# yuPeiyu98/Diffusion-Amortized-MCMC

Measured on AMD Instinct MI355X. Metric: Langevin z-steps/sec (B=128, z_dim=128, CIFAR-10), higher is better.
Workload: dtype f32; 1 GPU; cifar10 train-iteration Langevin block: 30 posterior steps on B=128 + 60 prior steps on 2B=256 split over the ranks (value counts posterior z-steps only); global_batch=128, per_rank_batch=128, per_rank_prior_chains=256, z_dim=128, ngf=128, posterior_steps=30, prior_steps=60, parallelism=dp1 (chains sharded, no collective)

## Files before the change

diffusion-amortized-mcmc_amd/csrc/gemm.hip:

```cpp
#include <algorithm>
#include <atomic>
#include <cstdlib>
#include <type_traits>

#include "gemm.h"

namespace damc {

constexpr int BN = 128;

template <int BK, int MT>
struct TileCfg {
  static constexpr int BM = 64 * MT;
  static constexpr int LDA = (BK == 16) ? BM + 2 : BM + 1;
  static constexpr int LDB = BN;
  static constexpr int AQ = BK / 4;
  static constexpr int AROWS_V = BM * BK / 1024;
  static constexpr int AROWS_S = BM * BK / 256;
  static constexpr int BROWS_V = BK / 8;
  static constexpr int BROWS_S = BK / 2;
};

template <int OM>
__device__ __forceinline__ long gemm_row_offset(const GemmArgs& p, int m, int py, int px) {
// ... 849 lines not shown
  hipLaunchKernelGGL((gemm_km_kernel<EPI, OM, PIPE, DBG>), dim3(ntm * ntn, 1, zdim), dim3(256), 0, s, a);
}

static int launch_gemm_km(const GemmArgs& a, Epi epi, OMode om, int zdim, hipStream_t s) {
  const int taps = a.Cg > 0 ? a.K / a.Cg : 0;
  if (!conv_kmajor_ok(a.Cg) || taps * a.Cg != a.K || a.kw <= 0 || taps % a.kw != 0 || taps > 32) return DAMC_ERR_ARG;
  if (om == O_PHASE && zdim != 4) return DAMC_ERR_ARG;
  if (om == O_DENSE && (a.k_per_z <= 0 || a.k_per_z % KM_BK != 0 ||
                        (long)zdim * a.k_per_z < a.K || (long)(zdim - 1) * a.k_per_z >= a.K))
    return DAMC_ERR_ARG;
  if (a.ldb < a.K || ((uintptr_t)a.A | (uintptr_t)a.B) % 16 != 0 || (a.ldb % 4) != 0) return DAMC_ERR_ARG;
  if ((double)a.N * a.ldb * 4 >= 2147483647.0) return DAMC_ERR_UNSUPPORTED;
  const long hwq = (long)a.Hq * a.Wq;
  if (a.M % hwq != 0) return DAMC_ERR_ARG;
  const long img = (long)a.Hin * a.Win * a.Cg;
  const long nimg = a.M / hwq;
  static const long lim = [] {
    const char* e = getenv("DAMC_KM_CHUNK_BYTES");
    const long v = e ? atol(e) : 0;
    return (v > 0 && v < 2147483647L) ? v : 2147483647L;
  }();
  const long per = (lim / 4 - 1) / img;
  if (per < 1) return DAMC_ERR_UNSUPPORTED;
  const long cimg = (om == O_PHASE) ? (long)a.Hout * a.Wout * a.ldc : hwq * a.ldc;
  for (long b0 = 0; b0 < nimg; b0 += per) {
    const long nb = std::min(per, nimg - b0);
    GemmArgs c = a;
    c.A = a.A + b0 * img;
    c.C = a.C + b0 * cimg;
    if (a.mask) c.mask = a.mask + b0 * cimg;
    c.M = (int)(nb * hwq);
    const char* esk = getenv("DAMC_KM_SKINNY");
    const char* ekr = getenv("DAMC_KM_SKINNY_ROWS");
    const int km_rows = ekr ? atoi(ekr) : 64;
    if (epi == EPI_STORE && om == O_DENSE && c.M <= km_rows && c.Hin == 1 && c.Win == 1 && c.Hq == 1 && c.Wq == 1 &&
        c.kw == 1 && c.Cg == c.K && !(esk && esk[0] == '0')) {
      const dim3 g((unsigned)zdim, (unsigned)((c.N + 127) / 128), (unsigned)((c.M + 31) / 32));
      hipLaunchKernelGGL(km_skinny_kernel, g, dim3(256), 0, s, c);
      continue;
    }
#define DAMC_KM(E_, O_)                \
  if (epi == E_ && om == O_) {         \
    launch_km_t<E_, O_>(c, zdim, s);   \
    continue;                          \
  }
    DAMC_KM(EPI_BIAS_ACT, O_PHASE)
    DAMC_KM(EPI_MASK, O_DENSE)
    DAMC_KM(EPI_BIAS_ACT, O_DENSE)
    DAMC_KM(EPI_STORE, O_DENSE)
#undef DAMC_KM
    return DAMC_ERR_UNSUPPORTED;
  }
  return (int)hipGetLastError();
}

constexpr int X3_BM = 256, X3_BN = 128, X3_BK = 32, X3_ROWB = 192;
__device__ __forceinline__ int x3_swz(int row) { return (row >> 1) & 3; }
constexpr int X3_F32A = 2097152, X3A_ROWB = 128;
constexpr int X3_NARROW = 4194304;
constexpr int X3_TAPSHARE = 16777216;
__device__ __forceinline__ int f32a_swz(int r) { return ((r >> 1) & 7) ^ ((((r >> 2) ^ (r >> 3)) & 1) << 1); }
__device__ __forceinline__ int ts_swz(int r) { return ((r >> 1) & 1) | (((r >> 2) & 1) << 2); }
static_assert(X3_NEGK % 32 == 0 && (X3_NEGK & (X3_NEGK - 1)) == 0, "sign blocks are whole K tiles, a power of two");
constexpr int X3_CHUNKS = 12;
typedef __bf16 bf16x8 __attribute__((ext_vector_type(8)));
typedef unsigned int u32x4 __attribute__((ext_vector_type(4)));

constexpr int X3_BASE = 261, X3_RASTER = 16, X3_WIDE = 524288, X3_KREG = 1048576;
constexpr int X3_BITS = X3_BASE | X3_RASTER | X3_WIDE | X3_KREG | X3_F32A | X3_NARROW | X3_TAPSHARE;
__device__ __forceinline__ void split3_octet(const float (&v)[8], bf16x8& h, bf16x8& m, bf16x8& l) {
#pragma unroll
  for (int e = 0; e < 8; ++e) {
    const __bf16 b0 = (__bf16)v[e];
    const float r1 = sub_rn(v[e], (float)b0);
    const __bf16 b1 = (__bf16)r1;
    const float r2 = sub_rn(r1, (float)b1);
    h[e] = b0;
    m[e] = b1;
    l[e] = (__bf16)r2;
  }
}

template <int NT>
__device__ __forceinline__ void proj16(const float* tile, int ts, int r0, int C, const float* w, int ldw,
                                       f32x4 (&acc)[NT]) {
  const int lane = threadIdx.x & 63, m = lane & 15, q = lane >> 4;
#pragma unroll
  for (int t = 0; t < NT; ++t) acc[t] = f32x4{0.f, 0.f, 0.f, 0.f};
  for (int g = 0; g < C / 16; ++g) {
    const f32x4 a = *reinterpret_cast<const f32x4*>(tile + (r0 + m) * ts + 16 * g + 4 * q);
#pragma unroll
    for (int t = 0; t < NT; ++t) {
      const f32x4 b = *reinterpret_cast<const f32x4*>(w + (long)(16 * t + m) * ldw + 16 * g + 4 * q);
#pragma unroll
      for (int e = 0; e < 4; ++e) acc[t] = __builtin_amdgcn_mfma_f32_16x16x4f32(a[e], b[e], acc[t], 0, 0, 0);
    }
  }
}

template <int NT>
__global__ __launch_bounds__(512) void proj_rows_kernel(const float* __restrict__ h, long npix, int C,
                                                        const float* __restrict__ w, int ldw, float* __restrict__ P,
                                                        long pstride) {
  constexpr int TS = 256 + 4;
  __shared__ __attribute__((aligned(16))) float tile[128 * TS];
  const int tid = threadIdx.x, wave = tid >> 6, lane = tid & 63;
  const long p0 = (long)blockIdx.x * 128;
  const int c4 = C / 4;
  for (int i = tid; i < 128 * c4; i += 512) {
    const int r = i / c4, c = (i - r * c4) * 4;
    const long pix = p0 + r;
    *reinterpret_cast<f32x4*>(tile + r * TS + c) =
        pix < npix ? *reinterpret_cast<const f32x4*>(h + pix * C + c) : f32x4{0.f, 0.f, 0.f, 0.f};
  }
  __syncthreads();
  const int m = lane & 15, q = lane >> 4;
  for (int c0 = 0; c0 < C; c0 += PROJ_CHUNK) {
    f32x4 acc[NT];
    proj16<NT>(tile + c0, TS, wave * 16, min(PROJ_CHUNK, C - c0), w + c0, ldw, acc);
    float* Pc = P + (c0 / PROJ_CHUNK) * pstride;
#pragma unroll
    for (int t = 0; t < NT; ++t)
#pragma unroll
      for (int r = 0; r < 4; ++r) {
        const long pix = p0 + wave * 16 + 4 * q + r;
        if (pix < npix) Pc[pix * (16 * NT) + 16 * t + m] = acc[t][r];
      }
  }
}

int launch_proj_rows(const float* h, long npix, int C, const float* w, int ldw, int np, float* P, long pstride,
                     hipStream_t s) {
  if (C <= 0 || C > 256 || C % 16 || (np != 32 && np != 64) || npix <= 0) return DAMC_ERR_ARG;
  if (C > PROJ_CHUNK && pstride < npix * np) return DAMC_ERR_ARG;
  const dim3 grid((unsigned)((npix + 127) / 128));
  if (np == 32)
    hipLaunchKernelGGL(proj_rows_kernel<2>, grid, dim3(512), 0, s, h, npix, C, w, ldw, P, pstride);
  else
    hipLaunchKernelGGL(proj_rows_kernel<4>, grid, dim3(512), 0, s, h, npix, C, w, ldw, P, pstride);
  return (int)hipGetLastError();
}

template <int EPI, int OM, int V = X3_BASE>
__global__ __launch_bounds__(512, (V & X3_NARROW) ? 2 : 1) void gemm_x3_kernel(GemmArgs p) {
  static_assert((V & X3_BASE) == X3_BASE && !(V & ~X3_BITS), "V: X3_BASE and the named variant bits only");
  constexpr bool WIDE = (V & X3_WIDE) != 0;
  constexpr bool NARROW = (V & X3_NARROW) != 0;
  static_assert(!NARROW || !(V & (X3_RASTER | X3_WIDE | X3_KREG | X3_F32A)), "NARROW: the default limb path, unsplit");
  constexpr int BM = WIDE ? 128 : NARROW ? 64 : X3_BM, BN = WIDE ? 256 : X3_BN;
  constexpr bool F32A = (V & X3_F32A) != 0;
  static_assert(!F32A || (OM != O_WGRAD && !WIDE), "F32A: 256 x 128 tiles, not the weight gradient");
  constexpr int AROWB = F32A ? X3A_ROWB : X3_ROWB, ESZ = F32A ? 4 : 6;
  constexpr int AJ = (BM * (F32A ? 8 : X3_CHUNKS) + 511) / 512, BJ = BN * X3_CHUNKS / 512;
  constexpr int BUFB = BM * AROWB + BN * X3_ROWB + ((V & X3_TAPSHARE) ? 2 * X3A_ROWB : 0);
  const int FLOG = __builtin_ctz((unsigned)p.negk >> 5), FLUSH = 1 << FLOG;
  __shared__ __attribute__((aligned(16))) unsigned char smem[2 * (BM + BN) * X3_ROWB];
  const int tid = threadIdx.x;
  const int lane = tid & 63;
  const int wave = tid >> 6;
  const int wm = (WIDE || NARROW) ? wave >> 2 : wave >> 1, wn = (WIDE || NARROW) ? wave & 3 : wave & 1;
  unsigned long long clk_t0 = 0, clk_r0 = 0;
  if (p.clk && tid == 0) {
    clk_t0 = __builtin_amdgcn_s_memtime();
    clk_r0 = __builtin_amdgcn_s_memrealtime();
  }
  constexpr bool RASTER = (V & X3_RASTER) != 0 && OM != O_WGRAD;
  const int wgid = xcd_remap(blockIdx.x, gridDim.x);
  const int ntn = (p.N + BN - 1) / BN;
  int tm, tn, z;
  if constexpr (RASTER) {
    const int nph = OM == O_PHASE ? 4 : 1;
    const int ntm = (p.M + BM - 1) / BM;
    int pr;
    supertile(wgid, ntm, ntn * nph, tm, pr);
    tn = pr / nph;
    z = pr - tn * nph;
  } else {
    tm = wgid / ntn;
    tn = wgid - tm * ntn;
    z = blockIdx.z;
  }
  const int m0 = tm * BM, n0 = tn * BN;

  int pad_y = p.pad_y, pad_x = p.pad_x, py = 0, px = 0;
  const unsigned short* Bg = p.B3;
  const bool KSPLIT = OM != O_WGRAD && p.ksplit > 1;
  constexpr bool KREG = (V & X3_KREG) != 0;
  static_assert(!KREG || !WIDE, "KREG: 256 x 128 tiles only");
  constexpr bool TSHARE = (V & X3_TAPSHARE) != 0;
  static_assert(!TSHARE || F32A, "TAPSHARE: the F32A path (on the slice-major walk)");
  const int nslz = KSPLIT ? p.ksplit / p.kbpw : 1;
  const int zph = KSPLIT ? z / nslz : z, zsl = KSPLIT ? z - zph * nslz : 0;
  if (OM == O_PHASE) {
    py = zph >> 1;
    px = zph & 1;
    pad_y = 1 - py;
    pad_x = 1 - px;
    Bg += (long)zph * p.b_zstride * 3;
  }
  int kbeg = 0, kend = p.K;
  if (KSPLIT) {
    kbeg = zsl * p.k_per_z;
    kend = min(p.K, kbeg + p.k_per_z);
  }
  if constexpr (OM == O_WGRAD) {
    const int nsl = gridDim.z / p.wg_phases;
    const int ph = z / nsl, sl = z - ph * nsl;
    if (p.wg_phases == 4) {
      py = ph >> 1;
      px = ph & 1;
      pad_y = 1 - py;
      pad_x = 1 - px;
    } else {
      pad_y = pad_x = 0;
    }
    Bg += (long)ph * p.b_zstride * 3;
    kbeg = sl * p.k_per_z;
    kend = min(p.K, kbeg + p.k_per_z);
  }
  const int Cg = p.Cg, kw = p.kw, Win = p.Win;
  const int kh = p.K / Cg / kw;
  const int nk = (OM == O_WGRAD || KSPLIT) ? max(kend - kbeg, 0) / X3_BK : p.K / X3_BK;
  const int kt0 = kbeg / X3_BK;
  const int hwq = p.Hq * p.Wq;
  const int nimg = (p.M + hwq - 1) / hwq;
  const __amdgpu_buffer_rsrc_t rsA = __builtin_amdgcn_make_buffer_rsrc(
      F32A ? (void*)p.A : (void*)p.A3, (short)0, (OM == O_WGRAD) ? Cg * p.K * 6 : nimg * p.Hin * Win * Cg * ESZ,
      0x00020000);
  const __amdgpu_buffer_rsrc_t rsB =
      __builtin_amdgcn_make_buffer_rsrc((void*)Bg, (short)0, p.N * p.K * 6, 0x00020000);

  int abase[AJ];
  unsigned amask[AJ], boff[BJ];
#pragma unroll
  for (int j = 0; j < AJ; ++j) {
    const int nch = F32A ? 8 : X3_CHUNKS;
    const int id = tid + 512 * j, row = id / nch, ch = id - row * nch;
    const int m = m0 + row;
    unsigned msk = 0;
    int base = 0;
    if constexpr (OM == O_WGRAD) {
      msk = 0xFFFFFFFFu;
      if (m < p.M) {
        const int t = m / Cg, ci = m - t * Cg;
        const int ty = t / kw, tx = t - ty * kw;
        const int dy = ty - pad_y, dx = tx - pad_x;
        base = ci * p.K + (dy * Win + dx) * p.wg_bp;
        msk = (unsigned)(dy + 1) | ((unsigned)(dx + 1) << 2);
      }
    } else if (m < p.M) {
      const int b = m / hwq;
      const int r = m - b * hwq;
      const int qy = r / p.Wq, qx = r - qy * p.Wq;
      const int iy0 = qy * p.stride - pad_y, ix0 = qx * p.stride - pad_x;
      base = ((b * p.Hin + iy0) * Win + ix0) * Cg;
      for (int ky = 0; ky < kh; ++ky)
        for (int kx = 0; kx < kw; ++kx)
          if ((unsigned)(iy0 + ky) < (unsigned)p.Hin && (unsigned)(ix0 + kx) < (unsigned)Win)
            msk |= 1u << (ky * kw + kx);
    }
    const int q = (ch / 3) ^ x3_swz(row), limb = ch - (ch / 3) * 3;
    abase[j] = F32A ? base * 4 + ((id & 7) ^ f32a_swz(row & 15)) * 16 : base * 6 + q * 48 + limb * 16;
    amask[j] = msk;
  }
#pragma unroll
  for (int j = 0; j < BJ; ++j) {
    const int id = tid + 512 * j, row = id / X3_CHUNKS, ch = id - row * X3_CHUNKS;
    const int q = (ch / 3) ^ x3_swz(row), limb = ch - (ch / 3) * 3;
    boff[j] = (unsigned)((n0 + row) * p.K * 6 + q * 48 + limb * 16);
  }

  int tap = 0, ci0 = 0, tky = 0, tkx = 0;
  const bool walk = OM != O_WGRAD && p.kwalk != 0;
  constexpr int WT = OM == O_PHASE ? 4 : 16;
  int wpos = 0;
  if (OM != O_WGRAD && kbeg > 0) {
    if (walk) {
      const int kt = kbeg / X3_BK;
      wpos = kt & (WT - 1);
      ci0 = (kt / WT) * X3_BK;
      tap = OM == O_PHASE ? wpos : x3_walk_tap(wpos);
    } else {
      tap = kbeg / Cg;
      ci0 = kbeg - tap * Cg;
    }
    tky = tap / kw;
    tkx = tap - tky * kw;
  }
  unsigned aoff[AJ];
  auto set_tap = [&]() {
    const int toff = (tky * Win + tkx) * Cg * ESZ;
#pragma unroll
    for (int j = 0; j < AJ; ++j) aoff[j] = ((amask[j] >> (tap & 31)) & 1u) ? (unsigned)(abase[j] + toff) : KM_OOB;
  };
  set_tap();
  auto next_ktile = [&]() {
    if (walk) {
      if (++wpos == WT) {
        wpos = 0;
        ci0 += X3_BK;
      }
      tap = OM == O_PHASE ? wpos : x3_walk_tap(wpos);
      tky = OM == O_PHASE ? tap >> 1 : tap >> 2;
      tkx = OM == O_PHASE ? tap & 1 : tap & 3;
      set_tap();
      return;
    }
    ci0 += X3_BK;
    if (ci0 == Cg) {
      ci0 = 0;
      ++tap;
      if (++tkx == kw) {
        tkx = 0;
        ++tky;
      }
      set_tap();
    }
  };
  typedef __attribute__((address_space(3))) void* lds_t;
  const int wbase = (tid & ~63) * 16;
  auto dma_ab = [&](int k0, int buf) {
    unsigned char* base = smem + buf * BUFB + wbase;
    if constexpr (OM == O_WGRAD) {
      const int pix = k0 / p.wg_bp;
      const int qy = pix / Win, qx = pix - qy * Win;
#pragma unroll
      for (int j = 0; j < AJ; ++j) {
        const int dy = (int)(amask[j] & 3u) - 1, dx = (int)((amask[j] >> 2) & 3u) - 1;
        const bool live = amask[j] != 0xFFFFFFFFu && (unsigned)(qy + dy) < (unsigned)p.Hin &&
                          (unsigned)(qx + dx) < (unsigned)Win;
        __builtin_amdgcn_raw_ptr_buffer_load_lds(rsA, (lds_t)(base + 512 * 16 * j), 16,
                                                 live ? (int)(abase[j] + k0 * 6) : (int)KM_OOB, 0, 0, 0);
      }
    } else {
#pragma unroll
      for (int j = 0; j < AJ; ++j)
        __builtin_amdgcn_raw_ptr_buffer_load_lds(rsA, (lds_t)(base + 512 * 16 * j), 16, (int)aoff[j], ci0 * ESZ, 0, 0);
    }
#pragma unroll
    for (int j = 0; j < BJ; ++j)
      __builtin_amdgcn_raw_ptr_buffer_load_lds(rsB, (lds_t)(base + BM * AROWB + 512 * 16 * j), 16, (int)boff[j],
                                               k0 * 6, 0, 0);
    if constexpr (OM != O_WGRAD) next_ktile();
  };

  f32x4 acc16[4][4], tot16[4][4];
#pragma unroll
  for (int i = 0; i < 4; ++i)
#pragma unroll
    for (int j = 0; j < 4; ++j) acc16[i][j] = tot16[i][j] = f32x4{0.f, 0.f, 0.f, 0.f};

  const int lrow = lane & 15, loct = lane >> 4;
  const int sw = x3_swz(lrow);
  const int afr = (wm * 64 + lrow) * X3_ROWB, bfr = (BM + wn * 64 + lrow) * X3_ROWB;
  const int oct16 = (loct ^ sw) * 48;

  auto flush16 = [&](int ktd) {
    const float sg = (p.b_negblk && (((ktd + kt0) >> FLOG) & 1)) ? -1.f : 1.f;
#pragma unroll
    for (int i = 0; i < 4; ++i)
#pragma unroll
      for (int j = 0; j < 4; ++j) {
#pragma unroll
        for (int r = 0; r < 4; ++r) tot16[i][j][r] = __builtin_fmaf(sg, acc16[i][j][r], tot16[i][j][r]);
        acc16[i][j] = f32x4{0.f, 0.f, 0.f, 0.f};
      }
  };
  if constexpr (NARROW) {
    auto dma_n = [&](int k0, int buf) {
      unsigned char* base = smem + buf * BUFB + wbase;
#pragma unroll
      for (int j = 0; j < AJ; ++j)
        if (512 * j + (tid & ~63) < BM * X3_CHUNKS)
          __builtin_amdgcn_raw_ptr_buffer_load_lds(rsA, (lds_t)(base + 512 * 16 * j), 16, (int)aoff[j], ci0 * 6, 0, 0);
#pragma unroll
      for (int j = 0; j < BJ; ++j)
        __builtin_amdgcn_raw_ptr_buffer_load_lds(rsB, (lds_t)(base + BM * X3_ROWB + 512 * 16 * j), 16, (int)boff[j],
                                                 k0 * 6, 0, 0);
      next_ktile();
    };
    if (nk > 0) dma_n(kbeg, 0);
    __syncthreads();
    const int afn = (wm * 32 + lrow) * X3_ROWB, bfn = (BM + wn * 32 + lrow) * X3_ROWB;
    for (int kt = 0; kt < nk; ++kt) {
      const unsigned char* base = smem + (kt & 1) * BUFB;
      if (kt + 1 < nk) dma_n(kbeg + (kt + 1) * X3_BK, (kt + 1) & 1);
      bf16x8 fa[2][3], fb[2][3];
#pragma unroll
      for (int t = 0; t < 2; ++t)
#pragma unroll
        for (int l = 0; l < 3; ++l) {
          fa[t][l] = *reinterpret_cast<const bf16x8*>(base + afn + t * 16 * X3_ROWB + oct16 + l * 16);
          fb[t][l] = *reinterpret_cast<const bf16x8*>(base + bfn + t * 16 * X3_ROWB + oct16 + l * 16);
        }
#pragma unroll
      for (int i = 0; i < 2; ++i)
#pragma unroll
        for (int j = 0; j < 2; ++j) {
          f32x4 c = acc16[i][j];
          c = __builtin_amdgcn_mfma_f32_16x16x32_bf16(fa[i][2], fb[j][0], c, 0, 0, 0);
          c = __builtin_amdgcn_mfma_f32_16x16x32_bf16(fa[i][1], fb[j][1], c, 0, 0, 0);
          c = __builtin_amdgcn_mfma_f32_16x16x32_bf16(fa[i][0], fb[j][2], c, 0, 0, 0);
          c = __builtin_amdgcn_mfma_f32_16x16x32_bf16(fa[i][1], fb[j][0], c, 0, 0, 0);
          c = __builtin_amdgcn_mfma_f32_16x16x32_bf16(fa[i][0], fb[j][1], c, 0, 0, 0);
          acc16[i][j] = __builtin_amdgcn_mfma_f32_16x16x32_bf16(fa[i][0], fb[j][0], c, 0, 0, 0);
        }
      __syncthreads();
      if (((kt + 1) & (FLUSH - 1)) == 0) {
        const float sg = (p.b_negblk && (((kt + kt0) >> FLOG) & 1)) ? -1.f : 1.f;
#pragma unroll
        for (int i = 0; i < 2; ++i)
#pragma unroll
          for (int j = 0; j < 2; ++j) {
#pragma unroll
            for (int r = 0; r < 4; ++r) tot16[i][j][r] = __builtin_fmaf(sg, acc16[i][j][r], tot16[i][j][r]);
            acc16[i][j] = f32x4{0.f, 0.f, 0.f, 0.f};
          }
      }
    }
  } else if constexpr (F32A) {
    auto dma_a = [&](int buf) {
      unsigned char* dst = smem + buf * BUFB + wbase;
#pragma unroll
      for (int j = 0; j < AJ; ++j)
        __builtin_amdgcn_raw_ptr_buffer_load_lds(rsA, (lds_t)(dst + 512 * 16 * j), 16, (int)aoff[j], ci0 * ESZ, 0, 0);
      next_ktile();
    };
    auto dma_b = [&](int k0, int buf) {
      unsigned char* dst = smem + buf * BUFB + BM * X3A_ROWB + wbase;
#pragma unroll
      for (int j = 0; j < BJ; ++j)
        __builtin_amdgcn_raw_ptr_buffer_load_lds(rsB, (lds_t)(dst + 512 * 16 * j), 16, (int)boff[j], k0 * 6, 0, 0);
    };
    const int fs = f32a_swz(lrow);
    const int ca0 = ((2 * loct) ^ fs) * 16, ca1 = ((2 * loct + 1) ^ fs) * 16;
    const int arow = (wave * 32 + lrow) * X3A_ROWB, brow = BM * X3A_ROWB + lrow * X3_ROWB + oct16;
    auto rd_a = [&](const unsigned char* buf, f32x4 (&av)[2][2]) {
#pragma unroll
      for (int a = 0; a < 2; ++a) {
        av[a][0] = *reinterpret_cast<const f32x4*>(buf + arow + a * 16 * X3A_ROWB + ca0);
        av[a][1] = *reinterpret_cast<const f32x4*>(buf + arow + a * 16 * X3A_ROWB + ca1);
      }
    };
    auto split2 = [&](const f32x4 (&av)[2][2], bf16x8 (&f)[2][3], int a, int e) {
#pragma unroll
      for (int d = 0; d < 2; ++d) {
        const float v = av[a][(e + d) >> 2][(e + d) & 3];
        const __bf16 b0 = (__bf16)v;
        const float r1 = sub_rn(v, (float)b0);
        const __bf16 b1 = (__bf16)r1;
        const float r2 = sub_rn(r1, (float)b1);
        f[a][0][e + d] = b0;
        f[a][1][e + d] = b1;
        f[a][2][e + d] = (__bf16)r2;
      }
    };
    auto rd_split = [&](const unsigned char* buf, bf16x8 (&f)[2][3]) {
      f32x4 av[2][2];
      rd_a(buf, av);
#pragma unroll
      for (int a = 0; a < 2; ++a)
#pragma unroll
        for (int e = 0; e < 8; e += 2) split2(av, f, a, e);
    };
    constexpr int ZREL = BM * AROWB + BN * X3_ROWB, TOFF = 2 * BUFB, NT = OM == O_PHASE ? 4 : 16;
    static_assert(!TSHARE || TOFF + NT * BM * 4 <= 2 * (BM + BN) * X3_ROWB, "no room for the read table");
    unsigned ts_ibase = 0;
    int ts_nv = 0, ts_pstr = 0, ts_o[2] = {0, 0};
    if constexpr (TSHARE) {
      const int r0 = tid >> 3, mi = m0 + r0;
      const unsigned b = mi / hwq, r = mi - b * hwq, qy = r / p.Wq, qx = r - qy * p.Wq;
      ts_ibase = ((b * p.Hin + qy * p.stride) * Win + qx * p.stride) * Cg * 4 + ((tid & 7) ^ ts_swz(r0)) * 16;
      ts_nv = min(4, max(0, (p.M - mi + 63) >> 6));
      ts_pstr = ((64 % hwq == 0) ? (64 / hwq) * p.Hin * Win : (64 / p.Wq) * p.stride * Win) * Cg * 4;
      for (int id = tid; id < NT * BM; id += 512) {
        const int row = id & (BM - 1), pos = id >> 8, m = m0 + row;
        int ky, kx, dlt;
        if constexpr (OM == O_PHASE) {
          ky = pos >> 1;
          kx = pos & 1;
          dlt = (ky - pad_y) * p.Wq + kx - pad_x;
        } else {
          const int c = pos >> 2, jj = pos & 3, tp = x3_walk_tap(pos);
          ky = tp >> 2;
          kx = tp & 3;
          dlt = ((jj >> 1) - 1 + (c >> 1)) * p.Wq + (jj & 1) - 1 + (c & 1);
        }
        const int bb = m / hwq, rr = m - bb * hwq, y = rr / p.Wq, x = rr - y * p.Wq;
        const int R = row + dlt;
        const bool live = m < p.M && (unsigned)(y * p.stride - pad_y + ky) < (unsigned)p.Hin &&
                          (unsigned)(x * p.stride - pad_x + kx) < (unsigned)Win && (unsigned)R < (unsigned)BM;
        reinterpret_cast<int*>(smem + TOFF)[id] = (live ? R * X3A_ROWB : ZREL + (R & 1) * X3A_ROWB) + ts_swz(R) * 16;
      }
      if (tid < 128) reinterpret_cast<float*>(smem + (tid >> 6) * BUFB + ZREL)[tid & 63] = 0.f;
    }
    auto dma_img = [&](int G, int j) {
      const int gg = (kt0 >> 2) + G;
      int sl = gg, coff = 0;
      if constexpr (OM == O_DENSE) {
        const int c = gg & 3;
        sl = gg >> 2;
        coff = ((1 - (c >> 1)) * Win + (1 - (c & 1))) * Cg * 4;
      }
      unsigned char* dst = smem + (G & 1) * BUFB + wbase + 512 * 16 * j;
      const int vo = j < ts_nv ? (int)(ts_ibase + (unsigned)(j * ts_pstr)) : (int)KM_OOB;
      __builtin_amdgcn_raw_ptr_buffer_load_lds(rsA, (lds_t)dst, 16, vo, sl * (X3_BK * 4) + coff, 0, 0);
    };
    const int ts_tb = TOFF + (wave * 32 + lrow) * 4;
    auto ts_addr = [&](int ktn) {
      const int ta = ts_tb + ((kt0 + ktn) & (NT - 1)) * (BM * 4), ib = ((ktn >> 2) & 1) * BUFB;
#pragma unroll
      for (int a = 0; a < 2; ++a) ts_o[a] = (*reinterpret_cast<const int*>(smem + ta + a * 64) ^ (loct << 5)) + ib;
    };
    auto rd_a_ts = [&](f32x4 (&av)[2][2]) {
#pragma unroll
      for (int a = 0; a < 2; ++a) {
        av[a][0] = *reinterpret_cast<const f32x4*>(smem + ts_o[a]);
        av[a][1] = *reinterpret_cast<const f32x4*>(smem + (ts_o[a] ^ 16));
      }
    };
    bf16x8 fx[2][3], fy[2][3], fb[2][3];
    if constexpr (TSHARE) {
      if (nk > 0) {
#pragma unroll
        for (int j = 0; j < 4; ++j) dma_img(0, j);
        dma_b(kbeg, 0);
      }
      if (nk > 4) dma_img(1, 0);
      __syncthreads();
      f32x4 av0[2][2];
      ts_addr(0);
      rd_a_ts(av0);
#pragma unroll
      for (int a = 0; a < 2; ++a)
#pragma unroll
        for (int e = 0; e < 8; e += 2) split2(av0, fx, a, e);
      ts_addr(1);
    } else {
      if (nk > 0) {
        dma_a(0);
        dma_b(kbeg, 0);
      }
      if (nk > 1) dma_a(1);
      __syncthreads();
      rd_split(smem, fx);
    }
    constexpr int SG_MFMA = 0x8, SG_VALU = 0x2, SG_DS_RD = 0x100;
    auto tile = [&](int kt, bf16x8 (&fc)[2][3], bf16x8 (&fn)[2][3]) {
      const unsigned char* base = smem + (kt & 1) * BUFB;
      if (kt + 1 < nk) dma_b(kbeg + (kt + 1) * X3_BK, (kt + 1) & 1);
      if constexpr (TSHARE) {
        const int G = ((kt + 1) >> 2) + 1;
        if (4 * G < nk) dma_img(G, (kt + 1) & 3);
      } else if (kt + 2 < nk) {
        dma_a(kt & 1);
      }
      f32x4 av[2][2];
      if constexpr (TSHARE)
        rd_a_ts(av);
      else
        rd_a(smem + ((kt + 1) & 1) * BUFB, av);
      auto rd_b = [&](int t, int slot) {
#pragma unroll
        for (int l = 0; l < 3; ++l) fb[slot][l] = *reinterpret_cast<const bf16x8*>(base + brow + t * 16 * X3_ROWB + l * 16);
      };
      rd_b(0, 0);
#pragma unroll
      for (int t = 0; t < 8; ++t) {
        if (t + 1 < 8) rd_b(t + 1, (t + 1) & 1);
        if constexpr (TSHARE) {
          if (t == 1) ts_addr(kt + 2);
        }
        const int sl = t & 1;
        split2(av, fn, t >> 2, (t & 3) * 2);
#pragma unroll
        for (int a = 0; a < 2; ++a) {
          f32x4 c = acc16[2 * a + (t >> 2)][t & 3];
          c = __builtin_amdgcn_mfma_f32_16x16x32_bf16(fc[a][2], fb[sl][0], c, 0, 0, 0);
          c = __builtin_amdgcn_mfma_f32_16x16x32_bf16(fc[a][1], fb[sl][1], c, 0, 0, 0);
          c = __builtin_amdgcn_mfma_f32_16x16x32_bf16(fc[a][0], fb[sl][2], c, 0, 0, 0);
          c = __builtin_amdgcn_mfma_f32_16x16x32_bf16(fc[a][1], fb[sl][0], c, 0, 0, 0);
          c = __builtin_amdgcn_mfma_f32_16x16x32_bf16(fc[a][0], fb[sl][1], c, 0, 0, 0);
          acc16[2 * a + (t >> 2)][t & 3] = __builtin_amdgcn_mfma_f32_16x16x32_bf16(fc[a][0], fb[sl][0], c, 0, 0, 0);
        }
      }
      __builtin_amdgcn_sched_group_barrier(SG_DS_RD, 10, 0);
#pragma unroll
      for (int t = 0; t < 8; ++t) {
#pragma unroll
        for (int m = 0; m < 12; ++m) {
          __builtin_amdgcn_sched_group_barrier(SG_MFMA, 1, 0);
          __builtin_amdgcn_sched_group_barrier(SG_VALU, 1, 0);
        }
        if (t + 2 < 8) __builtin_amdgcn_sched_group_barrier(SG_DS_RD, 3, 0);
        if constexpr (TSHARE) {
          if (t == 0) __builtin_amdgcn_sched_group_barrier(SG_DS_RD, 2, 0);
        }
      }
#pragma unroll
      for (int a = 0; a < 2; ++a)
#pragma unroll
        for (int l = 0; l < 3; ++l) asm volatile("" : "+v"(fn[a][l]));
      __syncthreads();
      if (((kt + 1) & (FLUSH - 1)) != 0) return;
      if constexpr (KREG) {
        const float sg = (p.b_negblk && (((kt + kt0) >> FLOG) & 1)) ? -1.f : 1.f;
        const int ntile = ((p.M + BM - 1) / BM) * ((p.N + BN - 1) / BN);
        const __amdgpu_buffer_rsrc_t rsl = __builtin_amdgcn_make_buffer_rsrc(
            (void*)(p.kslab + ((long)zph * p.ksplit + zsl * p.kbpw) * ntile * (BM * BN)), (short)0,
            p.kbpw * ntile * (BM * BN) * 4, 0x00020000);
        const int soff = ((kt >> FLOG) * ntile + tm * ntn + tn) * (BM * BN * 4);
        const int voff = ((wave >> 1) * 2 * 1024 + ((wave & 1) * 2) * 4 * 64 + lane) * 16;
#pragma unroll
        for (int i = 0; i < 4; ++i)
#pragma unroll
          for (int j = 0; j < 4; ++j) {
            const int a = i >> 1, wnp = i & 1;
            acc16[i][j] *= sg;
            if (m0 + wave * 32 + a * 16 < p.M) {
              __builtin_amdgcn_raw_buffer_store_b128(__builtin_bit_cast(u32x4, acc16[i][j]), rsl,
                                                     voff + soff + (wnp * 1024 + (a * 4 + j) * 64) * 16, 0, 0);
            }
            acc16[i][j] = f32x4{0.f, 0.f, 0.f, 0.f};
          }
      } else {
        flush16(kt);
      }
    };
    for (int kt = 0; kt < nk; kt += 2) {
      tile(kt, fx, fy);
      if (kt + 1 < nk) tile(kt + 1, fy, fx);
    }
  } else {
    if (nk > 0) dma_ab(kbeg, 0);
    __syncthreads();
    bf16x8 fa[4][3], fb[4][3];
    auto kloop = [&]() {
      for (int kt = 0; kt < nk; ++kt) {
        const unsigned char* base = smem + (kt & 1) * BUFB;
        if (kt + 1 < nk) dma_ab(kbeg + (kt + 1) * X3_BK, (kt + 1) & 1);
        auto rd_a = [&](int t) {
#pragma unroll
          for (int l = 0; l < 3; ++l) fa[t][l] = *reinterpret_cast<const bf16x8*>(base + afr + t * 16 * X3_ROWB + oct16 + l * 16);
        };
        auto rd_b = [&](int t) {
#pragma unroll
          for (int l = 0; l < 3; ++l) fb[t][l] = *reinterpret_cast<const bf16x8*>(base + bfr + t * 16 * X3_ROWB + oct16 + l * 16);
        };
        auto mf = [&](int i, int j) {
          f32x4 c = acc16[i][j];
          c = __builtin_amdgcn_mfma_f32_16x16x32_bf16(fa[i][2], fb[j][0], c, 0, 0, 0);
          c = __builtin_amdgcn_mfma_f32_16x16x32_bf16(fa[i][1], fb[j][1], c, 0, 0, 0);
          c = __builtin_amdgcn_mfma_f32_16x16x32_bf16(fa[i][0], fb[j][2], c, 0, 0, 0);
          c = __builtin_amdgcn_mfma_f32_16x16x32_bf16(fa[i][1], fb[j][0], c, 0, 0, 0);
          c = __builtin_amdgcn_mfma_f32_16x16x32_bf16(fa[i][0], fb[j][1], c, 0, 0, 0);
          acc16[i][j] = __builtin_amdgcn_mfma_f32_16x16x32_bf16(fa[i][0], fb[j][0], c, 0, 0, 0);
        };
        constexpr int SG_MFMA = 0x8, SG_DS_RD = 0x100;
        rd_a(0);
        rd_b(0);
        rd_b(1);
        mf(0, 0);
        rd_b(2);
        mf(0, 1);
        rd_b(3);
        mf(0, 2);
        rd_a(1);
        mf(0, 3);
        rd_a(2);
#pragma unroll
        for (int j = 0; j < 4; ++j) mf(1, j);
        rd_a(3);
#pragma unroll
        for (int i = 2; i < 4; ++i)
#pragma unroll
          for (int j = 0; j < 4; ++j) mf(i, j);
        __builtin_amdgcn_sched_group_barrier(SG_DS_RD, 9, 0);
        __builtin_amdgcn_sched_group_barrier(SG_MFMA, 6, 0);
        __builtin_amdgcn_sched_group_barrier(SG_DS_RD, 3, 0);
        __builtin_amdgcn_sched_group_barrier(SG_MFMA, 6, 0);
        __builtin_amdgcn_sched_group_barrier(SG_DS_RD, 3, 0);
        __builtin_amdgcn_sched_group_barrier(SG_MFMA, 6, 0);
        __builtin_amdgcn_sched_group_barrier(SG_DS_RD, 3, 0);
        __builtin_amdgcn_sched_group_barrier(SG_MFMA, 6, 0);
        __builtin_amdgcn_sched_group_barrier(SG_DS_RD, 3, 0);
        __builtin_amdgcn_sched_group_barrier(SG_MFMA, 24, 0);
        __builtin_amdgcn_sched_group_barrier(SG_DS_RD, 3, 0);
        __builtin_amdgcn_sched_group_barrier(SG_MFMA, 48, 0);
        __syncthreads();
        if (KREG) {
          if (((kt + 1) & (FLUSH - 1)) != 0) continue;
          const float sg = (p.b_negblk && (((kt + kt0) >> FLOG) & 1)) ? -1.f : 1.f;
          const int ntile = ((p.M + BM - 1) / BM) * ((p.N + BN - 1) / BN);
          const __amdgpu_buffer_rsrc_t rsl = __builtin_amdgcn_make_buffer_rsrc(
              (void*)(p.kslab + ((long)zph * p.ksplit + zsl * p.kbpw) * ntile * (BM * BN)), (short)0,
              p.kbpw * ntile * (BM * BN) * 4, 0x00020000);
          const int soff = ((kt >> FLOG) * ntile + tm * ntn + tn) * (BM * BN * 4);
          const int voff = (wave * 1024 + lane) * 16;
          const bool live = m0 + wm * 64 < p.M;
#pragma unroll
          for (int i = 0; i < 4; ++i)
#pragma unroll
            for (int j = 0; j < 4; ++j) {
              acc16[i][j] *= sg;
              if (live)
                __builtin_amdgcn_raw_buffer_store_b128(__builtin_bit_cast(u32x4, acc16[i][j]), rsl, voff,
                                                       soff + (i * 4 + j) * 1024, 0);
              acc16[i][j] = f32x4{0.f, 0.f, 0.f, 0.f};
            }
        } else if (((kt + 1) & (FLUSH - 1)) == 0) {
          flush16(kt);
        }
      }
    };
    kloop();
  }
  if (p.clk && tid == 0) {
    const unsigned long long t1 = __builtin_amdgcn_s_memtime(), r1 = __builtin_amdgcn_s_memrealtime();
    unsigned long long* c = p.clk + 4 * ((blockIdx.z * gridDim.x + blockIdx.x) % (unsigned)p.clk_n);
    c[0] = clk_t0;
    c[1] = clk_r0;
    c[2] = t1;
    c[3] = r1;
  }
  if (KREG) return;
  {
    const float sg = (p.b_negblk && nk > 0 && (((nk - 1 + kt0) >> FLOG) & 1)) ? -1.f : 1.f;
    constexpr int MI = NARROW ? 2 : 4;
#pragma unroll
    for (int i = 0; i < MI; ++i)
#pragma unroll
      for (int j = 0; j < MI; ++j)
#pragma unroll
        for (int r = 0; r < 4; ++r) acc16[i][j][r] = __builtin_fmaf(sg, acc16[i][j][r], tot16[i][j][r]);
  }
  constexpr int TS = BN + 4;
  static_assert(BM * TS * 4 + BM * 8 <= 2 * (BM + BN) * X3_ROWB, "epilogue tile exceeds the LDS");
  float* tile = reinterpret_cast<float*>(smem);
  long* rowtab = reinterpret_cast<long*>(smem + BM * TS * 4);
  float* Cz = p.C;
  if ((OM == O_DENSE || OM == O_WGRAD) && Cz) Cz += (long)(KSPLIT ? zph : z) * p.c_zstride;
  auto octet = [&](int row, int oct) {
    const int n = n0 + oct * 8;
    const long rowoff = rowtab[row];
    if (rowoff < 0 || n >= p.N) return;
    const long idx = rowoff + n;
    const f32x4 t0 = *reinterpret_cast<const f32x4*>(tile + row * TS + oct * 8);
    const f32x4 t1 = *reinterpret_cast<const f32x4*>(tile + row * TS + oct * 8 + 4);
    float v[8] = {t0.x, t0.y, t0.z, t0.w, t1.x, t1.y, t1.z, t1.w};
    if (EPI == EPI_BIAS_ACT) {
      if (p.bias) {
        const int nb = p.bias_mod < p.N ? n % p.bias_mod : n;
        const f32x4 b0 = *reinterpret_cast<const f32x4*>(p.bias + nb);
        const f32x4 b1 = *reinterpret_cast<const f32x4*>(p.bias + nb + 4);
        const float bb[8] = {b0.x, b0.y, b0.z, b0.w, b1.x, b1.y, b1.z, b1.w};
#pragma unroll
        for (int e = 0; e < 8; ++e) v[e] += bb[e];
      }
#pragma unroll
      for (int e = 0; e < 8; ++e) v[e] = act_apply(v[e], p.act, p.slope);
    } else if (EPI == EPI_MASK) {
      if (p.mask_sgn) {
        const unsigned bits = p.mask_sgn[idx >> 3];
#pragma unroll
        for (int e = 0; e < 8; ++e) v[e] *= ((bits >> e) & 1u) ? 1.f : p.mask_slope;
      } else {
        const f32x4 k0 = *reinterpret_cast<const f32x4*>(p.mask + idx);
        const f32x4 k1 = *reinterpret_cast<const f32x4*>(p.mask + idx + 4);
        const float kk[8] = {k0.x, k0.y, k0.z, k0.w, k1.x, k1.y, k1.z, k1.w};
#pragma unroll
        for (int e = 0; e < 8; ++e) v[e] *= act_grad_from_out(kk[e], p.mask_act, p.mask_slope);
      }
    }
    if (p.sgn) {
      unsigned bits = 0;
#pragma unroll
      for (int e = 0; e < 8; ++e) bits |= (v[e] > 0.f ? 1u : 0u) << e;
      p.sgn[idx >> 3] = (unsigned char)bits;
    }
    if (Cz && !p.proj_nostore) {
      *reinterpret_cast<f32x4*>(Cz + idx) = f32x4{v[0], v[1], v[2], v[3]};
      *reinterpret_cast<f32x4*>(Cz + idx + 4) = f32x4{v[4], v[5], v[6], v[7]};
    }
    if (p.C3) {
// ... 1188 lines not shown
```

Measured before the change: 59250 z-steps/s.

## Split the shared image tile into bf16 limbs once, reuse across taps

In the tap-sharing F32A path, each staged f32 image tile is now split into three bf16 limbs once, during the fourth phase of a four-tile group. The limbs are written to LDS and the other taps read them through the tap table, so they no longer redo the per-tap f32 read and VALU split. This changes the LDS layout (staging buffer, B double buffer, zero rows, table) and unrolls the k-loop by four with per-phase scheduling. The cost is more LDS, extra LDS writes, and more complex synchronisation, which could lower occupancy.

```diff
diff --git a/diffusion-amortized-mcmc_amd/csrc/gemm.hip b/diffusion-amortized-mcmc_amd/csrc/gemm.hip
--- a/diffusion-amortized-mcmc_amd/csrc/gemm.hip
+++ b/diffusion-amortized-mcmc_amd/csrc/gemm.hip
@@ -1025,9 +1025,15 @@
   static_assert(!F32A || (OM != O_WGRAD && !WIDE), "F32A: 256 x 128 tiles, not the weight gradient");
   constexpr int AROWB = F32A ? X3A_ROWB : X3_ROWB, ESZ = F32A ? 4 : 6;
   constexpr int AJ = (BM * (F32A ? 8 : X3_CHUNKS) + 511) / 512, BJ = BN * X3_CHUNKS / 512;
-  constexpr int BUFB = BM * AROWB + BN * X3_ROWB + ((V & X3_TAPSHARE) ? 2 * X3A_ROWB : 0);
+  constexpr int BUFB = BM * AROWB + BN * X3_ROWB;
+  constexpr int TS_NT = OM == O_PHASE ? 4 : 16;
+  constexpr int TS_STG = BM * X3_ROWB, TS_B = TS_STG + BM * X3A_ROWB, TS_ZERO = TS_B + 2 * BN * X3_ROWB;
+  constexpr int TS_TOFF = TS_ZERO + 4 * X3_ROWB, TS_END = TS_TOFF + TS_NT * BM * 4;
+  constexpr int SMEMB =
+      ((V & X3_TAPSHARE) && TS_END > 2 * (BM + BN) * X3_ROWB) ? TS_END : 2 * (BM + BN) * X3_ROWB;
+  static_assert(SMEMB <= 160 * 1024 && TS_ZERO % 256 == 0, "the LDS of a CU; zero rows on the images' bank phase");
   const int FLOG = __builtin_ctz((unsigned)p.negk >> 5), FLUSH = 1 << FLOG;
-  __shared__ __attribute__((aligned(16))) unsigned char smem[2 * (BM + BN) * X3_ROWB];
+  __shared__ __attribute__((aligned(16))) unsigned char smem[SMEMB];
   const int tid = threadIdx.x;
   const int lane = tid & 63;
   const int wave = tid >> 6;
@@ -1299,15 +1305,16 @@
         __builtin_amdgcn_raw_ptr_buffer_load_lds(rsA, (lds_t)(dst + 512 * 16 * j), 16, (int)aoff[j], ci0 * ESZ, 0, 0);
       next_ktile();
     };
+    constexpr int BOFF = TSHARE ? TS_B : BM * X3A_ROWB, BBUF = TSHARE ? BN * X3_ROWB : BUFB;
     auto dma_b = [&](int k0, int buf) {
-      unsigned char* dst = smem + buf * BUFB + BM * X3A_ROWB + wbase;
+      unsigned char* dst = smem + buf * BBUF + BOFF + wbase;
 #pragma unroll
       for (int j = 0; j < BJ; ++j)
         __builtin_amdgcn_raw_ptr_buffer_load_lds(rsB, (lds_t)(dst + 512 * 16 * j), 16, (int)boff[j], k0 * 6, 0, 0);
     };
     const int fs = f32a_swz(lrow);
     const int ca0 = ((2 * loct) ^ fs) * 16, ca1 = ((2 * loct + 1) ^ fs) * 16;
-    const int arow = (wave * 32 + lrow) * X3A_ROWB, brow = BM * X3A_ROWB + lrow * X3_ROWB + oct16;
+    const int arow = (wave * 32 + lrow) * X3A_ROWB, brow = BOFF + lrow * X3_ROWB + oct16;
     auto rd_a = [&](const unsigned char* buf, f32x4 (&av)[2][2]) {
 #pragma unroll
       for (int a = 0; a < 2; ++a) {
@@ -1336,11 +1343,10 @@
 #pragma unroll
         for (int e = 0; e < 8; e += 2) split2(av, f, a, e);
     };
-    constexpr int ZREL = BM * AROWB + BN * X3_ROWB, TOFF = 2 * BUFB, NT = OM == O_PHASE ? 4 : 16;
-    static_assert(!TSHARE || TOFF + NT * BM * 4 <= 2 * (BM + BN) * X3_ROWB, "no room for the read table");
     unsigned ts_ibase = 0;
-    int ts_nv = 0, ts_pstr = 0, ts_o[2] = {0, 0};
+    int ts_nv = 0, ts_pstr = 0;
     if constexpr (TSHARE) {
+      constexpr int NT = TS_NT;
       const int r0 = tid >> 3, mi = m0 + r0;
       const unsigned b = mi / hwq, r = mi - b * hwq, qy = r / p.Wq, qx = r - qy * p.Wq;
       ts_ibase = ((b * p.Hin + qy * p.stride) * Win + qx * p.stride) * Cg * 4 + ((tid & 7) ^ ts_swz(r0)) * 16;
@@ -1363,9 +1369,9 @@
         const int R = row + dlt;
         const bool live = m < p.M && (unsigned)(y * p.stride - pad_y + ky) < (unsigned)p.Hin &&
                           (unsigned)(x * p.stride - pad_x + kx) < (unsigned)Win && (unsigned)R < (unsigned)BM;
-        reinterpret_cast<int*>(smem + TOFF)[id] = (live ? R * X3A_ROWB : ZREL + (R & 1) * X3A_ROWB) + ts_swz(R) * 16;
-      }
-      if (tid < 128) reinterpret_cast<float*>(smem + (tid >> 6) * BUFB + ZREL)[tid & 63] = 0.f;
+        reinterpret_cast<int*>(smem + TS_TOFF)[id] = (live ? R * X3_ROWB : TS_ZERO + (R & 3) * X3_ROWB) + x3_swz(R) * 16;
+      }
+      if (tid < 4 * X3_ROWB / 4) reinterpret_cast<float*>(smem + TS_ZERO)[tid] = 0.f;
     }
     auto dma_img = [&](int G, int j) {
       const int gg = (kt0 >> 2) + G;
@@ -1375,107 +1381,48 @@
         sl = gg >> 2;
         coff = ((1 - (c >> 1)) * Win + (1 - (c & 1))) * Cg * 4;
       }
-      unsigned char* dst = smem + (G & 1) * BUFB + wbase + 512 * 16 * j;
+      unsigned char* dst = smem + TS_STG + wbase + 512 * 16 * j;
       const int vo = j < ts_nv ? (int)(ts_ibase + (unsigned)(j * ts_pstr)) : (int)KM_OOB;
       __builtin_amdgcn_raw_ptr_buffer_load_lds(rsA, (lds_t)dst, 16, vo, sl * (X3_BK * 4) + coff, 0, 0);
     };
-    const int ts_tb = TOFF + (wave * 32 + lrow) * 4;
-    auto ts_addr = [&](int ktn) {
-      const int ta = ts_tb + ((kt0 + ktn) & (NT - 1)) * (BM * 4), ib = ((ktn >> 2) & 1) * BUFB;
-#pragma unroll
-      for (int a = 0; a < 2; ++a) ts_o[a] = (*reinterpret_cast<const int*>(smem + ta + a * 64) ^ (loct << 5)) + ib;
+    const int ts_tb = TS_TOFF + (wave * 32 + lrow) * 4;
+    auto ts_addr = [&](int ktn, int (&o)[2]) {
+      const int ta = ts_tb + ((kt0 + ktn) & (TS_NT - 1)) * (BM * 4);
+#pragma unroll
+      for (int a = 0; a < 2; ++a) o[a] = *reinterpret_cast<const int*>(smem + ta + a * 64) ^ (loct << 4);
     };
-    auto rd_a_ts = [&](f32x4 (&av)[2][2]) {
+    auto rd_limb = [&](const int (&o)[2], bf16x8 (&f)[2][3], int a, int l) {
+      f[a][l] = *reinterpret_cast<const bf16x8*>(smem + o[a] + l * 64);
+    };
+    const int cv_rd = TS_STG + (wave * 32 + lrow) * X3A_ROWB + ((2 * loct) ^ ts_swz(lrow)) * 16;
+    auto rd_stg = [&](f32x4 (&av)[2][2]) {
 #pragma unroll
       for (int a = 0; a < 2; ++a) {
-        av[a][0] = *reinterpret_cast<const f32x4*>(smem + ts_o[a]);
-        av[a][1] = *reinterpret_cast<const f32x4*>(smem + (ts_o[a] ^ 16));
-      }
+        av[a][0] = *reinterpret_cast<const f32x4*>(smem + cv_rd + a * 16 * X3A_ROWB);
+        av[a][1] = *reinterpret_cast<const f32x4*>(smem + (cv_rd ^ 16) + a * 16 * X3A_ROWB);
+      }
+    };
+    const int cv_wr = (wave * 32 + lrow) * X3_ROWB + (loct ^ sw) * 16;
+    auto wr_limb = [&](const bf16x8 (&f)[2][3], int a) {
+#pragma unroll
+      for (int l = 0; l < 3; ++l) *reinterpret_cast<bf16x8*>(smem + cv_wr + a * 16 * X3_ROWB + l * 64) = f[a][l];
     };
     bf16x8 fx[2][3], fy[2][3], fb[2][3];
-    if constexpr (TSHARE) {
-      if (nk > 0) {
-#pragma unroll
-        for (int j = 0; j < 4; ++j) dma_img(0, j);
-        dma_b(kbeg, 0);
-      }
-      if (nk > 4) dma_img(1, 0);
-      __syncthreads();
-      f32x4 av0[2][2];
-      ts_addr(0);
-      rd_a_ts(av0);
-#pragma unroll
-      for (int a = 0; a < 2; ++a)
-#pragma unroll
-        for (int e = 0; e < 8; e += 2) split2(av0, fx, a, e);
-      ts_addr(1);
-    } else {
-      if (nk > 0) {
-        dma_a(0);
-        dma_b(kbeg, 0);
-      }
-      if (nk > 1) dma_a(1);
-      __syncthreads();
-      rd_split(smem, fx);
-    }
-    constexpr int SG_MFMA = 0x8, SG_VALU = 0x2, SG_DS_RD = 0x100;
-    auto tile = [&](int kt, bf16x8 (&fc)[2][3], bf16x8 (&fn)[2][3]) {
-      const unsigned char* base = smem + (kt & 1) * BUFB;
-      if (kt + 1 < nk) dma_b(kbeg + (kt + 1) * X3_BK, (kt + 1) & 1);
-      if constexpr (TSHARE) {
-        const int G = ((kt + 1) >> 2) + 1;
-        if (4 * G < nk) dma_img(G, (kt + 1) & 3);
-      } else if (kt + 2 < nk) {
-        dma_a(kt & 1);
-      }
-      f32x4 av[2][2];
-      if constexpr (TSHARE)
-        rd_a_ts(av);
-      else
-        rd_a(smem + ((kt + 1) & 1) * BUFB, av);
-      auto rd_b = [&](int t, int slot) {
-#pragma unroll
-        for (int l = 0; l < 3; ++l) fb[slot][l] = *reinterpret_cast<const bf16x8*>(base + brow + t * 16 * X3_ROWB + l * 16);
-      };
-      rd_b(0, 0);
-#pragma unroll
-      for (int t = 0; t < 8; ++t) {
-        if (t + 1 < 8) rd_b(t + 1, (t + 1) & 1);
-        if constexpr (TSHARE) {
-          if (t == 1) ts_addr(kt + 2);
-        }
-        const int sl = t & 1;
-        split2(av, fn, t >> 2, (t & 3) * 2);
-#pragma unroll
-        for (int a = 0; a < 2; ++a) {
-          f32x4 c = acc16[2 * a + (t >> 2)][t & 3];
-          c = __builtin_amdgcn_mfma_f32_16x16x32_bf16(fc[a][2], fb[sl][0], c, 0, 0, 0);
-          c = __builtin_amdgcn_mfma_f32_16x16x32_bf16(fc[a][1], fb[sl][1], c, 0, 0, 0);
-          c = __builtin_amdgcn_mfma_f32_16x16x32_bf16(fc[a][0], fb[sl][2], c, 0, 0, 0);
-          c = __builtin_amdgcn_mfma_f32_16x16x32_bf16(fc[a][1], fb[sl][0], c, 0, 0, 0);
-          c = __builtin_amdgcn_mfma_f32_16x16x32_bf16(fc[a][0], fb[sl][1], c, 0, 0, 0);
-          acc16[2 * a + (t >> 2)][t & 3] = __builtin_amdgcn_mfma_f32_16x16x32_bf16(fc[a][0], fb[sl][0], c, 0, 0, 0);
-        }
-      }
-      __builtin_amdgcn_sched_group_barrier(SG_DS_RD, 10, 0);
-#pragma unroll
-      for (int t = 0; t < 8; ++t) {
-#pragma unroll
-        for (int m = 0; m < 12; ++m) {
-          __builtin_amdgcn_sched_group_barrier(SG_MFMA, 1, 0);
-          __builtin_amdgcn_sched_group_barrier(SG_VALU, 1, 0);
-        }
-        if (t + 2 < 8) __builtin_amdgcn_sched_group_barrier(SG_DS_RD, 3, 0);
-        if constexpr (TSHARE) {
-          if (t == 0) __builtin_amdgcn_sched_group_barrier(SG_DS_RD, 2, 0);
-        }
-      }
-#pragma unroll
-      for (int a = 0; a < 2; ++a)
-#pragma unroll
-        for (int l = 0; l < 3; ++l) asm volatile("" : "+v"(fn[a][l]));
-      __syncthreads();
-      if (((kt + 1) & (FLUSH - 1)) != 0) return;
+    constexpr int SG_MFMA = 0x8, SG_VALU = 0x2, SG_DS_RD = 0x100, SG_DS_WR = 0x200;
+    auto mfma6 = [&](const bf16x8 (&fc)[2][3], int t) {
+      const int sl = t & 1;
+#pragma unroll
+      for (int a = 0; a < 2; ++a) {
+        f32x4 c = acc16[2 * a + (t >> 2)][t & 3];
+        c = __builtin_amdgcn_mfma_f32_16x16x32_bf16(fc[a][2], fb[sl][0], c, 0, 0, 0);
+        c = __builtin_amdgcn_mfma_f32_16x16x32_bf16(fc[a][1], fb[sl][1], c, 0, 0, 0);
+        c = __builtin_amdgcn_mfma_f32_16x16x32_bf16(fc[a][0], fb[sl][2], c, 0, 0, 0);
+        c = __builtin_amdgcn_mfma_f32_16x16x32_bf16(fc[a][1], fb[sl][0], c, 0, 0, 0);
+        c = __builtin_amdgcn_mfma_f32_16x16x32_bf16(fc[a][0], fb[sl][1], c, 0, 0, 0);
+        acc16[2 * a + (t >> 2)][t & 3] = __builtin_amdgcn_mfma_f32_16x16x32_bf16(fc[a][0], fb[sl][0], c, 0, 0, 0);
+      }
+    };
+    auto flush_blk = [&](int kt) {
       if constexpr (KREG) {
         const float sg = (p.b_negblk && (((kt + kt0) >> FLOG) & 1)) ? -1.f : 1.f;
         const int ntile = ((p.M + BM - 1) / BM) * ((p.N + BN - 1) / BN);
@@ -1500,9 +1447,134 @@
         flush16(kt);
       }
     };
-    for (int kt = 0; kt < nk; kt += 2) {
-      tile(kt, fx, fy);
-      if (kt + 1 < nk) tile(kt + 1, fy, fx);
+    if constexpr (TSHARE) {
+      int oa[2], ob[2];
+      if (nk > 0) {
+#pragma unroll
+        for (int j = 0; j < 4; ++j) dma_img(0, j);
+        dma_b(kbeg, 0);
+      }
+      __syncthreads();
+      {
+        f32x4 av0[2][2];
+        rd_stg(av0);
+#pragma unroll
+        for (int a = 0; a < 2; ++a) {
+#pragma unroll
+          for (int e = 0; e < 8; e += 2) split2(av0, fx, a, e);
+          wr_limb(fx, a);
+        }
+      }
+      ts_addr(0, oa);
+      ts_addr(1, ob);
+      __syncthreads();
+      auto tile = [&](int kt, auto PH_, bf16x8 (&fc)[2][3], bf16x8 (&fn)[2][3], int (&on)[2], int (&of)[2]) {
+        constexpr int PH = decltype(PH_)::value;
+        const unsigned char* base = smem + (PH & 1) * BBUF;
+        if (kt + 1 < nk) dma_b(kbeg + (kt + 1) * X3_BK, (PH + 1) & 1);
+        if constexpr (PH < 3) {
+          const int G = (kt >> 2) + 1;
+          if (4 * G < nk) {
+            if constexpr (PH == 0) dma_img(G, 0);
+            dma_img(G, PH + 1);
+          }
+        }
+        auto rd_b = [&](int t, int slot) {
+#pragma unroll
+          for (int l = 0; l < 3; ++l) fb[slot][l] = *reinterpret_cast<const bf16x8*>(base + brow + t * 16 * X3_ROWB + l * 16);
+        };
+        f32x4 av[2][2];
+        if constexpr (PH == 0) {
+#pragma unroll
+          for (int i = 0; i < 6; ++i) rd_limb(of, fc, i / 3, i % 3);
+        }
+        if constexpr (PH == 3) rd_stg(av);
+        rd_b(0, 0);
+        rd_b(1, 1);
+#pragma unroll
+        for (int t = 0; t < 8; ++t) {
+          if constexpr (PH == 3) split2(av, fn, t >> 2, (t & 3) * 2);
+          mfma6(fc, t);
+          if (t + 2 < 8) rd_b(t + 2, t & 1);
+          if constexpr (PH < 3) {
+            if (t < 6) rd_limb(on, fn, t / 3, t % 3);
+          }
+          if (t == 0) ts_addr(kt + 2, of);
+          if constexpr (PH == 3) {
+            if (t == 4) wr_limb(fn, 0);
+            if (t == 7) wr_limb(fn, 1);
+          }
+        }
+        __builtin_amdgcn_sched_group_barrier(SG_DS_RD, PH == 0 ? 12 : PH == 3 ? 10 : 6, 0);
+#pragma unroll
+        for (int t = 0; t < 8; ++t) {
+#pragma unroll
+          for (int m = 0; m < 12; ++m) {
+            __builtin_amdgcn_sched_group_barrier(SG_MFMA, 1, 0);
+            if constexpr (PH == 3) __builtin_amdgcn_sched_group_barrier(SG_VALU, 1, 0);
+          }
+          if (t + 2 < 8) __builtin_amdgcn_sched_group_barrier(SG_DS_RD, 3, 0);
+          if (PH < 3 && t < 6) __builtin_amdgcn_sched_group_barrier(SG_DS_RD, 1, 0);
+          if (t == 0) __builtin_amdgcn_sched_group_barrier(SG_DS_RD, 2, 0);
+          if (PH == 3 && (t == 4 || t == 7)) __builtin_amdgcn_sched_group_barrier(SG_DS_WR, 3, 0);
+        }
+        __syncthreads();
+        if constexpr (PH == 3) {
+          if (((kt + 1) & (FLUSH - 1)) == 0) flush_blk(kt);
+        }
+      };
+      for (int kt = 0; kt < nk; kt += 4) {
+        tile(kt, std::integral_constant<int, 0>{}, fx, fy, ob, oa);
+        tile(kt + 1, std::integral_constant<int, 1>{}, fy, fx, oa, ob);
+        tile(kt + 2, std::integral_constant<int, 2>{}, fx, fy, ob, oa);
+        tile(kt + 3, std::integral_constant<int, 3>{}, fy, fx, ob, ob);
+      }
+    } else {
+      if (nk > 0) {
+        dma_a(0);
+        dma_b(kbeg, 0);
+      }
+      if (nk > 1) dma_a(1);
+      __syncthreads();
+      rd_split(smem, fx);
+      auto tile = [&](int kt, bf16x8 (&fc)[2][3], bf16x8 (&fn)[2][3]) {
+        const unsigned char* base = smem + (kt & 1) * BUFB;
+        if (kt + 1 < nk) dma_b(kbeg + (kt + 1) * X3_BK, (kt + 1) & 1);
+        if (kt + 2 < nk) dma_a(kt & 1);
+        f32x4 av[2][2];
+        rd_a(smem + ((kt + 1) & 1) * BUFB, av);
+        auto rd_b = [&](int t, int slot) {
+#pragma unroll
+          for (int l = 0; l < 3; ++l) fb[slot][l] = *reinterpret_cast<const bf16x8*>(base + brow + t * 16 * X3_ROWB + l * 16);
+        };
+        rd_b(0, 0);
+#pragma unroll
+        for (int t = 0; t < 8; ++t) {
+          if (t + 1 < 8) rd_b(t + 1, (t + 1) & 1);
+          split2(av, fn, t >> 2, (t & 3) * 2);
+          mfma6(fc, t);
+        }
+        __builtin_amdgcn_sched_group_barrier(SG_DS_RD, 10, 0);
+#pragma unroll
+        for (int t = 0; t < 8; ++t) {
+#pragma unroll
+          for (int m = 0; m < 12; ++m) {
+            __builtin_amdgcn_sched_group_barrier(SG_MFMA, 1, 0);
+            __builtin_amdgcn_sched_group_barrier(SG_VALU, 1, 0);
+          }
+          if (t + 2 < 8) __builtin_amdgcn_sched_group_barrier(SG_DS_RD, 3, 0);
+        }
+#pragma unroll
+        for (int a = 0; a < 2; ++a)
+#pragma unroll
+          for (int l = 0; l < 3; ++l) asm volatile("" : "+v"(fn[a][l]));
+        __syncthreads();
+        if (((kt + 1) & (FLUSH - 1)) == 0) flush_blk(kt);
+      };
+      for (int kt = 0; kt < nk; kt += 2) {
+        tile(kt, fx, fy);
+        if (kt + 1 < nk) tile(kt + 1, fy, fx);
+      }
     }
   } else {
     if (nk > 0) dma_ab(kbeg, 0);
```

Result: faster. 60640 z-steps/s, median of 6 (+2.4%).
